# NilFoundation/crypto3-zk

Measured on AMD Instinct MI355X. Metric: MSM Mpoints/sec, BLS12-381 G1 Pippenger, 2^20 points per GPU, higher is better.
Workload: dtype u32; 1 GPU; BLS12-381 G1 Pippenger MSM, ONE MSM of 1 x 2^20 random points/scalars, bases resident; points_per_gpu=1048576, parallelism=point-range partition x1 + one all-gather of the 144-B partial sums

## Files before the change

__graft_entry__.py:

```python
import importlib.util
import os
import subprocess
import sys

ROOT = os.path.dirname(os.path.abspath(__file__))


def _load_pkg():
    if "crypto3_zk_amd" in sys.modules:
        return sys.modules["crypto3_zk_amd"]
    pkg_dir = os.path.join(ROOT, "crypto3-zk_amd")
    spec = importlib.util.spec_from_file_location("crypto3_zk_amd", os.path.join(pkg_dir, "__init__.py"),
                                                  submodule_search_locations=[pkg_dir])
    mod = importlib.util.module_from_spec(spec)
    sys.modules["crypto3_zk_amd"] = mod
    spec.loader.exec_module(mod)
    return mod


def build() -> None:
    env = dict(os.environ)
    subprocess.check_call(["make", "-C", os.path.join(ROOT, "crypto3-zk_amd"), "-j4", "all"], env=env)
    subprocess.check_call(["make", "-C", os.path.join(ROOT, "oracle"), "liboracle.so"], env=env)
    subprocess.check_call(["make", "-j2", "-C", os.path.join(ROOT, "tests", "cpp")], env=env)
    subprocess.check_call(["make", "-C", os.path.join(ROOT, "tests", "cpp"), "-f", "merkle.mk"], env=env)
    subprocess.check_call(["make", "-C", os.path.join(ROOT, "tests", "cpp"), "-f", "pow.mk"], env=env)
    subprocess.check_call(["make", "-j2", "-C", os.path.join(ROOT, "tests", "cpp"), "-f", "pasta.mk"], env=env)
    subprocess.check_call(["make", "-C", os.path.join(ROOT, "tests", "cpp"), "-f", "ipa.mk"], env=env)
    zk = _load_pkg()
    zk.load_library()


def smoke() -> None:
    import numpy as np

    sys.path.insert(0, os.path.join(ROOT, "oracle"))
    import cport as cp
    import pyoracle as po

    zk = _load_pkg()
    ctx = zk.Context(0)
    n = 5000
    ks = cp.random_fr(0, 1, n)
    bases = ctx.bases_from_scalars(zk.BLS12_381, zk.G1, ks)
    pts, inf = bases.download()
    exp_pts, _ = cp.batch_mul(0, 1, ks)
    assert (pts == exp_pts).all(), "device fixed-base multiples differ from the oracle"
    sc = cp.random_fr(0, 2, n)
    aff, is_inf = ctx.msm_affine(bases, sc)
    exp, einf = cp.msm(0, 1, pts, sc, chunks=2)
    assert is_inf == einf and (aff == exp).all(), "MSM differs from the oracle"
    grp = zk.DeviceGroup([0, 0])
    gb = grp.upload_bases(zk.BLS12_381, zk.G1, pts)
    gaff, ginf = grp.msm_affine(gb, sc)
    assert ginf == einf and (gaff == exp).all(), "device-group MSM differs from the oracle"
    gb.free()
    grp.close()
    k2 = cp.random_fr(0, 4, 300)
    b2 = ctx.bases_from_scalars(zk.BLS12_381, zk.G2, k2)
    p2, _ = b2.download()
    s2 = cp.random_fr(0, 5, 300)
    aff2, inf2 = ctx.msm_affine(b2, s2)
    exp2, einf2 = cp.msm(0, 2, p2, s2, chunks=2)
    assert inf2 == einf2 and (aff2 == exp2).all(), "G2 MSM differs from the oracle"
    b2.free()
    log_m = 12
    w = np.array(po.to_limbs(po.BLS12_381.root_of_unity(log_m), 4), dtype=np.uint64)
    a = cp.random_fr(0, 3, 2 << log_m).reshape(2, 1 << log_m, 4)
    got = ctx.ntt(zk.BLS12_381, a, log_m, w)
    assert (got == cp.ntt(0, a, log_m, w)).all(), "NTT differs from the oracle"
    assert (ctx.ntt(zk.BLS12_381, got, log_m, w, inverse=True) == a).all()
    bases.free()
    M, nin = 1024, 10
    g16 = cp.Groth16(0, M, nin, seed=3)
    kind, m = cp.domain_choice(M + nin + 1, 32)
    wd = np.array(po.to_limbs(po.BLS12_381.root_of_unity((M + nin).bit_length()), 4), dtype=np.uint64)
    gen = np.array(po.to_limbs(po.BLS12_381.fr_generator, 4), dtype=np.uint64)
    g16.set_domain(kind, m, wd)
    r1cs = ctx.upload_r1cs(zk.BLS12_381, g16.M, g16.n, g16.N, g16.csr(0), g16.csr(1), g16.csr(2))
    assert (r1cs.kind, r1cs.m) == (kind, m) == (2, 1040), "the constraint system's domain is not the reference's choice"
    z = np.concatenate([np.array([[1, 0, 0, 0]], dtype=np.uint64), g16.assignment()])
    assert (ctx.groth16_witness_h(r1cs, z, wd, gen) == g16.witness_map(wd, gen)).all(), "witness map over the step domain differs from the oracle"
    r1cs.free()
    import hashlib
    state = hashlib.sha256(b"zkhip smoke").digest()
    k = next(k for k in range(1 << 20)
             if int.from_bytes(hashlib.sha256(hashlib.sha256(state + (12345 + k).to_bytes(4, "big")).digest()).digest()[28:], "big") & 0xFFF == 0)
    assert ctx.pow_grind(state, 12345, 0xFFF) == (12345 + k, k + 1), "the device's proof of work is not the first accepted nonce"
    ctx.close()
    print("smoke ok: G1 MSM n=5000 (one context and a device group of two), G2 MSM n=300, NTT 2^12 x 2 and the witness map over a step radix-2 domain bit-exact against the oracle; proof of work (12 bits) = the reference loop's nonce")


if __name__ == "__main__":
    build()
    if len(sys.argv) > 1 and sys.argv[1] == "smoke":
        smoke()
```

crypto3-zk_amd/csrc/msm_core.hpp:

```cpp
#pragma once
#include <algorithm>
#include <string>
#include <type_traits>
#include <vector>

#ifndef ZK_NOINLINE_MUL2
#define ZK_NOINLINE_MUL2 1
#endif
#include "ctx.hpp"
#include "curve.hpp"
#include "msm_ops.hpp"
#include "msm_recode.hpp"
#include "msm_bucket_acc.hpp"
#include "fu_pair.hpp"
#include "fu_quad.hpp"

namespace {

using namespace zkhip;

constexpr uint32_t MSM_LARGE_BUCKET = 128;
constexpr uint32_t MSM_LARGE_CHUNK = 4096;
#ifndef MSM_G1_THREADS
#define MSM_G1_THREADS 64
#endif
#ifndef MSM_G2_THREADS
#define MSM_G2_THREADS 256
#endif
#ifndef MSM_G2_WAVES
#define MSM_G2_WAVES 2
#endif

template <uint32_t THREADS>
ZK_D void block_inclusive_scan(uint32_t *scratch) {
    const uint32_t t = threadIdx.x;
    __syncthreads();
    for (uint32_t d = 1; d < THREADS; d <<= 1) {
        uint32_t x = t >= d ? scratch[t - d] : 0;
        __syncthreads();
        scratch[t] += x;
        __syncthreads();
    }
}

__global__ __launch_bounds__(256) void msm_scan_local(const uint32_t *__restrict__ hist, uint32_t count, uint32_t *__restrict__ offs,
                                                      uint32_t *__restrict__ block_sums) {
    __shared__ uint32_t part[256];
    const uint32_t t = threadIdx.x, base = blockIdx.x * 1024 + t * 4;
    uint32_t v[4], s = 0;
#pragma unroll
    for (int k = 0; k < 4; ++k) {
        v[k] = base + k < count ? hist[base + k] : 0;
        s += v[k];
    }
    part[t] = s;
    block_inclusive_scan<256>(part);
    uint32_t run = part[t] - s;
#pragma unroll
    for (int k = 0; k < 4; ++k) {
        if (base + k < count) offs[base + k] = run;
        run += v[k];
    }
    if (t == 255) block_sums[blockIdx.x] = part[255];
}

__global__ __launch_bounds__(1024) void msm_scan_top(uint32_t *__restrict__ block_sums, uint32_t nblocks, uint32_t *__restrict__ total) {
    __shared__ uint32_t part[1024];
    const uint32_t t = threadIdx.x;
    const uint32_t per = (nblocks + 1023) / 1024;
    const uint32_t lo = min(nblocks, t * per), hi = min(nblocks, lo + per);
    uint32_t s = 0;
    for (uint32_t i = lo; i < hi; ++i) s += block_sums[i];
    part[t] = s;
    block_inclusive_scan<1024>(part);
    uint32_t run = part[t] - s;
    for (uint32_t i = lo; i < hi; ++i) {
        uint32_t x = block_sums[i];
        block_sums[i] = run;
        run += x;
    }
    if (t == 1023) *total = part[1023];
}

__global__ __launch_bounds__(256) void msm_scan_add(uint32_t *__restrict__ offs, uint32_t count, const uint32_t *__restrict__ block_sums,
                                                    uint32_t *__restrict__ cursor) {
    const uint32_t base = blockIdx.x * 1024 + threadIdx.x * 4;
    const uint32_t add = block_sums[blockIdx.x];
#pragma unroll
    for (int k = 0; k < 4; ++k) {
        if (base + k < count) {
            uint32_t x = offs[base + k] + add;
            offs[base + k] = x;
            cursor[base + k] = x;
        }
    }
}

__global__ __launch_bounds__(1024) void msm_scan_single(const uint32_t *__restrict__ hist, uint32_t count, uint32_t *__restrict__ offs,
                                                        uint32_t *__restrict__ cursor) {
    __shared__ uint32_t part[1024];
    __shared__ uint32_t carry;
    const uint32_t t = threadIdx.x;
    if (t == 0) carry = 0;
    __syncthreads();
    for (uint32_t base = 0; base < count; base += 1024) {
        const uint32_t v = base + t < count ? hist[base + t] : 0;
        part[t] = v;
        block_inclusive_scan<1024>(part);
        const uint32_t excl = carry + part[t] - v;
        if (base + t < count) {
            offs[base + t] = excl;
            if (cursor != offs) cursor[base + t] = excl;
        }
        __syncthreads();
        if (t == 1023) carry += part[1023];
        __syncthreads();
    }
    if (t == 0) offs[count] = carry;
}
constexpr uint32_t MSM_SCAN_SINGLE_MAX = 1u << 16;

inline int msm_scan(zkhip_ctx *ctx, const char *name, const uint32_t *hist, uint32_t count, uint32_t *offs, uint32_t *bsums) {
    if (count <= MSM_SCAN_SINGLE_MAX) {
        ZK_LAUNCH(ctx, name, msm_scan_single, dim3(1), dim3(1024), 0, hist, count, offs, offs);
        return 0;
    }
    const uint32_t nblk = (count + 1023) / 1024;
    ZK_LAUNCH(ctx, name, msm_scan_local, dim3(nblk), dim3(256), 0, hist, count, offs, bsums);
    ZK_LAUNCH(ctx, name, msm_scan_top, dim3(1), dim3(1024), 0, bsums, nblk, offs + count);
    ZK_LAUNCH(ctx, name, msm_scan_add, dim3(nblk), dim3(256), 0, offs, count, bsums, offs);
    return 0;
}

template <class FR>
__global__ __launch_bounds__(256) void msm_digits_only(const uint32_t *__restrict__ scalars, uint32_t n, MsmWindows win, uint32_t wrank,
                                                       uint32_t wworld, uint32_t *__restrict__ dig) {
    uint32_t i = blockIdx.x * blockDim.x + threadIdx.x;
    if (i >= n) return;
    uint32_t s[8];
    const uint32_t flip = msm_fold_scalar<FR>(scalars + (size_t)i * 8, s) ? 0x80000000u : 0u;
    uint32_t carry = 0, next = wrank, lw = 0;
    for (int w = 0; w < win.W; ++w) {
        uint32_t d = msm_recode(s, win.off(w), win.width(w), carry);
        if ((uint32_t)w != next) continue;
        dig[(size_t)lw * n + i] = d == DIG_NONE ? d : d ^ flip;
        next += wworld;
        ++lw;
    }
}

struct SortGeom {
    uint32_t n;
    uint32_t W;
    uint32_t B;
    uint32_t S;
    uint32_t lowb;
    uint32_t nsuper;
    uint32_t tile;
    uint32_t ntile;
    uint32_t slot0;
    uint32_t tables;
    uint32_t bases_n;
    uint32_t base_off;
};
struct SortBig {
    static constexpr uint32_t TILE = 16384, THREADS = 1024;
};
struct SortSmall {
// ... 273 lines not shown
    constexpr int NL = FieldOps<F>::WORDS;
    uint32_t g = (blockIdx.x * blockDim.x + threadIdx.x) / LPB;
    if (g >= q * B) return;
    const uint32_t s = g / B;
    uint32_t *dst = buckets + (size_t)g * (4 * NL);
    XYZZ<F> acc = xyzz_load<F>(dst);
    for (uint32_t k = 1; k < 4; ++k)
        if (s + k * q < cur) acc = xyzz_add(acc, xyzz_load<F>(buckets + ((size_t)g + (size_t)k * q * B) * (4 * NL)));
    xyzz_store<F>(dst, acc);
}

constexpr int MSM_TAIL_THREADS = 256;

template <class F>
ZK_D XYZZ<F> block_tree_sum(uint32_t *lds, XYZZ<F> acc, uint32_t t, uint32_t nthreads) {
    constexpr int NL = FieldOps<F>::WORDS;
    xyzz_store<F>(lds + (size_t)t * (4 * NL), acc);
    __syncthreads();
    for (uint32_t d = nthreads / 2; d >= 1; d >>= 1) {
        if (t < d) {
            acc = xyzz_add(xyzz_load<F>(lds + (size_t)t * (4 * NL)), xyzz_load<F>(lds + (size_t)(t + d) * (4 * NL)));
            xyzz_store<F>(lds + (size_t)t * (4 * NL), acc);
        }
        __syncthreads();
    }
    return acc;
}

template <class F, int LPB>
#ifndef ZK_TAIL_WAVES
#define ZK_TAIL_WAVES 2
#endif
__global__ __launch_bounds__(MSM_TAIL_THREADS, ZK_TAIL_WAVES) void msm_bucket_red(const uint32_t *__restrict__ buckets, uint32_t B, uint32_t L, uint32_t nseg,
                                                                   uint32_t nblk, uint32_t *__restrict__ partial) {
    constexpr int NL = FieldOps<F>::WORDS;
    extern __shared__ __attribute__((aligned(16))) uint32_t lds[];
    constexpr uint32_t SLOTS = MSM_TAIL_THREADS / LPB;
    const uint32_t t = threadIdx.x / LPB, w = blockIdx.x / nblk, seg = (blockIdx.x % nblk) * SLOTS + t;
    XYZZ<F> sum = XYZZ<F>::infinity();
    if (seg < nseg) {
        const uint32_t *base = buckets + ((size_t)w * B + (size_t)seg * L) * (4 * NL);
        if (L == 1) {
            sum = xyzz_mul_small(xyzz_load<F>(base), seg + 1);
        } else {
            XYZZ<F> run = XYZZ<F>::infinity();
            for (int b = (int)L - 1; b >= 0; --b) {
                run = xyzz_add(run, xyzz_load<F>(base + (size_t)b * (4 * NL)));
                sum = xyzz_add(sum, run);
            }
            if (seg != 0) sum = xyzz_add(sum, xyzz_mul_small(run, seg * L));
        }
    }
    sum = block_tree_sum<F>(lds, sum, t, SLOTS);
    if (t == 0) xyzz_store<F>(partial + (size_t)blockIdx.x * (4 * NL), sum);
}

template <class F, int LPB>
__global__ __launch_bounds__(256) void msm_window_sum(const uint32_t *__restrict__ partial, uint32_t nblk, uint32_t *__restrict__ winsum) {
    constexpr int NL = FieldOps<F>::WORDS;
    extern __shared__ __attribute__((aligned(16))) uint32_t lds[];
    const uint32_t w = blockIdx.x, t = threadIdx.x / LPB, slots = blockDim.x / LPB;
    XYZZ<F> acc = XYZZ<F>::infinity();
    for (uint32_t j = t; j < nblk; j += slots) acc = xyzz_add(acc, xyzz_load<F>(partial + ((size_t)w * nblk + j) * (4 * NL)));
    if (nblk > 1) acc = block_tree_sum<F>(lds, acc, t, slots);
    if (t == 0) xyzz_store<F>(winsum + (size_t)w * (4 * NL), acc);
}
inline uint32_t msm_window_threads(uint32_t nblk, int lanes_per_point) { return (size_t)nblk * lanes_per_point > 128 ? 256u : 64u; }

struct MsmFold {
    uint32_t B, C, R, log_c;
    uint32_t run;
    uint32_t m_row, m_col;
};
inline MsmFold msm_fold_geom(const zkhip_ctx *ctx, uint32_t B) {
    MsmFold g;
    int lb = 0;
    while ((1u << lb) < B) ++lb;
    g.B = B;
    g.log_c = (uint32_t)((lb + 1) / 2);
    g.C = 1u << g.log_c;
    g.R = B >> g.log_c;
    g.run = ctx->opt_msm_fold_run > 0 ? (uint32_t)ctx->opt_msm_fold_run : (B >= (1u << 18) ? 8u : 4u);
    g.run = std::max(1u, std::min(g.run, g.R));
    g.m_row = g.C / g.run;
    g.m_col = g.R / g.run;
    return g;
}

template <class FA, int LA, class FT, int LT>
__global__ __launch_bounds__(MSM_TAIL_THREADS, ZK_TAIL_WAVES) void msm_fold(const uint32_t *__restrict__ buckets, MsmFold g, uint32_t *__restrict__ level2) {
    constexpr int NL = FieldOps<FA>::WORDS;
    constexpr uint32_t SA = MSM_TAIL_THREADS / LA, ST = MSM_TAIL_THREADS / LT, PW = 4 * NL;
    extern __shared__ __attribute__((aligned(16))) uint32_t lds[];
    const uint32_t half_wgs = g.B / (SA * g.run);
    const uint32_t w = blockIdx.x / (2 * half_wgs), k = blockIdx.x % (2 * half_wgs);
    const bool col = k >= half_wgs;
    const uint32_t wg = col ? k - half_wgs : k, s = threadIdx.x / LA;
    const uint32_t m = col ? g.m_col : g.m_row, G = SA / m;
    uint32_t first, stride, slot;
    if (!col) {
        first = (wg * G + s / m) * g.C + s % m;
        stride = m;
        slot = s;
    } else {
        const uint32_t j = s / G, ll = s % G;
        first = j * g.C + wg * G + ll;
        stride = m * g.C;
        slot = ll * m + j;
    }
    {
        const uint32_t *src = buckets + ((size_t)w * g.B + first) * PW;
        XYZZ<FA> acc = xyzz_load<FA>(src);
        for (uint32_t i = 1; i < g.run; ++i) acc = xyzz_add(acc, xyzz_load<FA>(src + (size_t)i * stride * PW));
        xyzz_store<FA>(lds + (size_t)slot * PW, acc);
    }
    __syncthreads();
    const uint32_t t = threadIdx.x / LT;
    for (uint32_t half = m / 2; half >= 1; half >>= 1) {
        const uint32_t adds = G * half;
        for (uint32_t idx = t; idx < adds; idx += ST) {
            uint32_t *p = lds + (size_t)((idx / half) * m + idx % half) * PW;
            xyzz_store<FT>(p, xyzz_add(xyzz_load<FT>(p), xyzz_load<FT>(p + (size_t)half * PW)));
        }
        __syncthreads();
    }
    for (uint32_t i = t; i < G; i += ST) {
        const uint32_t o = wg * G + i;
        if (col || o != 0)
            xyzz_store<FT>(level2 + (((size_t)2 * w + (col ? 0 : 1)) * g.C + (col ? o : o - 1)) * PW, xyzz_load<FT>(lds + (size_t)i * m * PW));
    }
}

template <class F>
ZK_D void xyzz_store_canonical_jacobian(uint32_t *dst, const XYZZ<F> &p) {
    constexpr int CW = FieldOps<F>::CANON_WORDS;
    Jacobian<F> j = xyzz_to_jacobian(p);
    FieldOps<F>::to_canonical(dst, j.X);
    FieldOps<F>::to_canonical(dst + CW, j.Y);
    FieldOps<F>::to_canonical(dst + 2 * CW, j.Z);
}

template <class F, int LPB>
__global__ __launch_bounds__(64) void msm_final_fold(const uint32_t *__restrict__ winsum, uint32_t count, uint32_t shift, uint32_t *const *__restrict__ outs,
                                                     uint32_t *__restrict__ out) {
    constexpr int NL = FieldOps<F>::WORDS;
    if (blockIdx.x >= count || threadIdx.x >= LPB) return;
    XYZZ<F> acc = xyzz_load<F>(winsum + ((size_t)2 * blockIdx.x + 1) * (4 * NL));
    if (!acc.is_inf())
        for (uint32_t i = 0; i < shift; ++i) acc = xyzz_dbl(acc);
    acc = xyzz_add(acc, xyzz_load<F>(winsum + (size_t)2 * blockIdx.x * (4 * NL)));
    xyzz_store_canonical_jacobian<F>(outs ? outs[blockIdx.x] : out, acc);
}

template <class F, int LPB>
__global__ __launch_bounds__(64) void msm_final(const uint32_t *__restrict__ winsum, int W, MsmWindows win, uint32_t *__restrict__ out_jac) {
    constexpr int NL = FieldOps<F>::WORDS;
    if (blockIdx.x != 0 || threadIdx.x >= LPB) return;
    XYZZ<F> acc = XYZZ<F>::infinity();
    for (int w = W - 1; w >= 0; --w) {
        if (!acc.is_inf())
            for (int i = 0; i < win.width(w); ++i) acc = xyzz_dbl(acc);
        acc = xyzz_add(acc, xyzz_load<F>(winsum + (size_t)w * (4 * NL)));
    }
    xyzz_store_canonical_jacobian<F>(out_jac, acc);
}

template <class F>
__global__ __launch_bounds__(256) void bases_to_mont(const uint32_t *__restrict__ canon, const uint8_t *__restrict__ inf, uint32_t n,
                                                     uint32_t *__restrict__ pts) {
    typedef FieldOps<F> O;
    uint32_t i = blockIdx.x * blockDim.x + threadIdx.x;
    if (i >= n) return;
    const uint32_t *c = canon + (size_t)i * (2 * O::CANON_WORDS);
    Affine<F> a;
    if (inf != nullptr && inf[i]) a = Affine<F>::infinity();
    else a = {O::from_canonical(c), O::from_canonical(c + O::CANON_WORDS)};
    affine_store<F>(pts + (size_t)i * (2 * O::WORDS), a);
}

template <class F>
__global__ __launch_bounds__(256) void bases_from_mont(const uint32_t *__restrict__ pts, uint32_t n, uint32_t *__restrict__ out,
                                                       uint8_t *__restrict__ inf) {
    typedef FieldOps<F> O;
    uint32_t i = blockIdx.x * blockDim.x + threadIdx.x;
    if (i >= n) return;
    Affine<F> a = affine_load<F>(pts + (size_t)i * (2 * O::WORDS));
    inf[i] = a.is_inf() ? 1 : 0;
    uint32_t *o = out + (size_t)i * (2 * O::CANON_WORDS);
    O::to_canonical(o, a.x);
    O::to_canonical(o + O::CANON_WORDS, a.y);
}

template <class F>
__global__ __launch_bounds__(64) void bases_mul(uint32_t *__restrict__ pts, const uint32_t *__restrict__ base_canonical,
                                                const uint32_t *__restrict__ scalars, uint32_t n) {
    constexpr int NL = FieldOps<F>::WORDS;
    uint32_t i = blockIdx.x * blockDim.x + threadIdx.x;
    if (i >= n) return;
    Affine<F> g = {FieldOps<F>::from_canonical(base_canonical), FieldOps<F>::from_canonical(base_canonical + FieldOps<F>::CANON_WORDS)};
    const uint32_t *s = scalars + (size_t)i * 8;
    XYZZ<F> acc = XYZZ<F>::infinity();
    for (int b = 255; b >= 0; --b) {
        acc = xyzz_dbl(acc);
        if ((s[b >> 5] >> (b & 31)) & 1) acc = xyzz_madd(acc, g);
    }
    affine_store<F>(pts + (size_t)i * (2 * NL), xyzz_to_affine(acc));
}

constexpr int FIXED_WBITS = 8, FIXED_NW = 32, FIXED_ROW = 1 << FIXED_WBITS;
template <class F>
__global__ __launch_bounds__(64) void bases_fixed_table(const uint32_t *__restrict__ base_canonical, uint32_t *__restrict__ tab, uint32_t *__restrict__ tmp) {
    typedef FieldOps<F> O;
    constexpr int NL = O::WORDS;
    const uint32_t w = blockIdx.x * blockDim.x + threadIdx.x;
    if (w >= FIXED_NW) return;
    Affine<F> g = {O::from_canonical(base_canonical), O::from_canonical(base_canonical + O::CANON_WORDS)};
    XYZZ<F> P = XYZZ<F>::from_affine(g);
    for (uint32_t k = 0; k < w * FIXED_WBITS; ++k) P = xyzz_dbl(P);
    uint32_t *mine = tmp + (size_t)w * FIXED_ROW * (5 * NL);
    XYZZ<F> acc = P;
    F pre = F::one();
    for (uint32_t d = 1; d < FIXED_ROW; ++d) {
        if (d > 1) acc = xyzz_add(acc, P);
        uint32_t *slot = mine + (size_t)d * (5 * NL);
        xyzz_store<F>(slot, acc);
        pre = O::mul(pre, O::mul(acc.ZZ, acc.ZZZ));
        O::store(slot + 4 * NL, pre);
    }
    F inv = O::inv(pre);
    for (uint32_t d = FIXED_ROW; d-- > 1;) {
        const uint32_t *slot = mine + (size_t)d * (5 * NL);
        XYZZ<F> q = xyzz_load<F>(slot);
        F before = d > 1 ? O::load(mine + (size_t)(d - 1) * (5 * NL) + 4 * NL) : F::one();
        F dinv = O::mul(inv, before);
        inv = O::mul(inv, O::mul(q.ZZ, q.ZZZ));
        Affine<F> a = {O::mul(q.X, O::mul(dinv, q.ZZZ)), O::mul(q.Y, O::mul(dinv, q.ZZ))};
        affine_store<F>(tab + ((size_t)w * FIXED_ROW + d) * (2 * NL), a);
    }
}
constexpr uint32_t FIXED_CHUNK = 8;
template <class F>
__global__ __launch_bounds__(64) void bases_mul_fixed(uint32_t *__restrict__ pts, const uint32_t *__restrict__ tab, const uint32_t *__restrict__ scalars,
                                                      uint32_t n, uint32_t *__restrict__ tmp) {
    typedef FieldOps<F> O;
    constexpr int NL = O::WORDS;
    const uint32_t lo = (blockIdx.x * blockDim.x + threadIdx.x) * FIXED_CHUNK;
    if (lo >= n) return;
    const uint32_t cnt = n - lo < FIXED_CHUNK ? n - lo : FIXED_CHUNK;
    F pre = F::one();
    for (uint32_t k = 0; k < cnt; ++k) {
        const uint32_t *s = scalars + (size_t)(lo + k) * 8;
        XYZZ<F> acc = XYZZ<F>::infinity();
        for (uint32_t w = 0; w < FIXED_NW; ++w) {
            const uint32_t d = (s[w >> 2] >> ((w & 3) * 8)) & 0xFFu;
            if (d) acc = xyzz_madd(acc, affine_load<F>(tab + ((size_t)w * FIXED_ROW + d) * (2 * NL)));
        }
        uint32_t *slot = tmp + (size_t)(lo + k) * (5 * NL);
        xyzz_store<F>(slot, acc);
        if (!acc.is_inf()) pre = O::mul(pre, O::mul(acc.ZZ, acc.ZZZ));
        O::store(slot + 4 * NL, pre);
    }
    F inv = O::inv(pre);
    for (uint32_t k = cnt; k-- > 0;) {
        const uint32_t *slot = tmp + (size_t)(lo + k) * (5 * NL);
        XYZZ<F> q = xyzz_load<F>(slot);
        if (q.is_inf()) {
            affine_store<F>(pts + (size_t)(lo + k) * (2 * NL), Affine<F>::infinity());
            continue;
        }
        F before = k > 0 ? O::load(tmp + (size_t)(lo + k - 1) * (5 * NL) + 4 * NL) : F::one();
        F dinv = O::mul(inv, before);
        inv = O::mul(inv, O::mul(q.ZZ, q.ZZZ));
        Affine<F> a = {O::mul(q.X, O::mul(dinv, q.ZZZ)), O::mul(q.Y, O::mul(dinv, q.ZZ))};
        affine_store<F>(pts + (size_t)(lo + k) * (2 * NL), a);
    }
}

template <class F>
__global__ __launch_bounds__(64) void bases_precompute_range(uint32_t *__restrict__ pts, uint32_t n, uint32_t lo, uint32_t cnt, MsmWindows win,
                                                             uint32_t wrank, uint32_t wworld, uint32_t *__restrict__ tmp) {
    const int W = win.W;
    typedef FieldOps<F> O;
    constexpr int NL = O::WORDS;
    uint32_t j = blockIdx.x * blockDim.x + threadIdx.x;
    if (j >= cnt) return;
    const uint32_t i = lo + j;
    const uint32_t extra = wrank != 0 ? 1u : 0u;
    auto slot_ptr = [&](uint32_t w) { return pts + ((size_t)(w / wworld + extra) * n + i) * (2 * NL); };
    Affine<F> p = affine_load<F>(pts + (size_t)i * (2 * NL));
    if (p.is_inf()) {
        for (uint32_t w = (wrank != 0 ? wrank : wworld); w < (uint32_t)W; w += wworld) affine_store<F>(slot_ptr(w), Affine<F>::infinity());
        return;
    }
    XYZZ<F> acc = XYZZ<F>::from_affine(p);
    F pre = F::one();
    uint32_t kept = 0;
    for (int w = 1; w < W; ++w) {
        for (int k = 0; k < win.width(w - 1); ++k) acc = xyzz_dbl(acc);
        if ((uint32_t)w % wworld != wrank) continue;
        uint32_t *slot = tmp + ((size_t)kept * cnt + j) * (5 * NL);
        xyzz_store<F>(slot, acc);
        pre = O::mul(pre, O::mul(acc.ZZ, acc.ZZZ));
        O::store(slot + 4 * NL, pre);
        ++kept;
    }
    if (kept == 0) return;
    F inv = O::inv(pre);
    uint32_t w = ((uint32_t)(W - 1) - wrank) / wworld * wworld + wrank;
    for (uint32_t k = kept; k-- > 0; w -= wworld) {
        const uint32_t *slot = tmp + ((size_t)k * cnt + j) * (5 * NL);
        XYZZ<F> q = xyzz_load<F>(slot);
        F before = k > 0 ? O::load(tmp + ((size_t)(k - 1) * cnt + j) * (5 * NL) + 4 * NL) : F::one();
        F dinv = O::mul(inv, before);
        inv = O::mul(inv, O::mul(q.ZZ, q.ZZZ));
        Affine<F> a = {O::mul(q.X, O::mul(dinv, q.ZZZ)), O::mul(q.Y, O::mul(dinv, q.ZZ))};
        affine_store<F>(slot_ptr(w), a);
    }
}

template <class F>
__global__ void jac_to_affine_k(const uint32_t *__restrict__ jac, uint32_t *__restrict__ aff, uint8_t *__restrict__ inf) {
    typedef FieldOps<F> O;
    constexpr int CW = O::CANON_WORDS;
    if (blockIdx.x != 0 || threadIdx.x != 0) return;
    Jacobian<F> j = {O::from_canonical(jac), O::from_canonical(jac + CW), O::from_canonical(jac + 2 * CW)};
    XYZZ<F> q = xyzz_from_jacobian(j);
    inf[0] = q.is_inf() ? 1 : 0;
    Affine<F> a = xyzz_to_affine(q);
    O::to_canonical(aff, a.x);
    O::to_canonical(aff + CW, a.y);
}

template <class F>
__global__ void jac_sum_k(const uint32_t *__restrict__ jac, uint32_t count, uint32_t *__restrict__ out) {
    typedef FieldOps<F> O;
    constexpr int CW = O::CANON_WORDS;
    if (blockIdx.x != 0 || threadIdx.x != 0) return;
    XYZZ<F> acc = XYZZ<F>::infinity();
    for (uint32_t i = 0; i < count; ++i) {
        const uint32_t *p = jac + (size_t)i * 3 * CW;
        Jacobian<F> j = {O::from_canonical(p), O::from_canonical(p + CW), O::from_canonical(p + 2 * CW)};
        acc = xyzz_add(acc, xyzz_from_jacobian(j));
    }
    Jacobian<F> r = xyzz_to_jacobian(acc);
    O::to_canonical(out, r.X);
    O::to_canonical(out + CW, r.Y);
    O::to_canonical(out + 2 * CW, r.Z);
}

template <class F>
__global__ void msm_write_infinity(uint32_t *out_jac) {
    if (blockIdx.x != 0 || threadIdx.x != 0) return;
    xyzz_store_canonical_jacobian<F>(out_jac, XYZZ<F>::infinity());
}

template <class F, int LPB>
__global__ __launch_bounds__(64) void msm_final_batch(const uint32_t *__restrict__ winsum, uint32_t count, uint32_t *const *__restrict__ outs) {
    constexpr int NL = FieldOps<F>::WORDS;
    constexpr int CW = FieldOps<F>::CANON_WORDS;
    if (blockIdx.x >= count || threadIdx.x >= LPB) return;
    Jacobian<F> j = xyzz_to_jacobian(xyzz_load<F>(winsum + (size_t)blockIdx.x * (4 * NL)));
    uint32_t *out = outs[blockIdx.x];
    FieldOps<F>::to_canonical(out, j.X);
    FieldOps<F>::to_canonical(out + CW, j.Y);
    FieldOps<F>::to_canonical(out + 2 * CW, j.Z);
}


inline uint32_t msm_tail_segment(const zkhip_ctx *ctx, uint32_t B, size_t sets, int lanes_per_point) {
    uint32_t L = 1;
    if (ctx->opt_msm_segment_log >= 0) L = 1u << std::min(ctx->opt_msm_segment_log, 8);
    else {
        const size_t lanes = sets * B * (size_t)lanes_per_point;
        while (L < 16 && lanes / L > 65536) L <<= 1;
        while (L < 64 && lanes / L > 262144) L <<= 1;
    }
    return std::min(B, L);
}

struct MsmTailGeom {
    uint32_t L, nseg;
    uint32_t slots, nblk;
    uint32_t wthreads;
    size_t lds_red, lds_win;
};
template <class Lane>
MsmTailGeom msm_tail_geom(const zkhip_ctx *ctx, uint32_t B, size_t sets) {
    constexpr size_t point_bytes = (size_t)4 * FieldOps<typename Lane::type>::WORDS * 4;
    constexpr int XL = Lane::LANES;
    MsmTailGeom t;
    t.L = msm_tail_segment(ctx, B, sets, XL);
    t.nseg = B / t.L;
    t.slots = MSM_TAIL_THREADS / XL;
    t.nblk = (t.nseg + t.slots - 1) / t.slots;
    t.wthreads = msm_window_threads(t.nblk, XL);
    t.lds_red = t.slots * point_bytes;
    t.lds_win = t.wthreads / XL * point_bytes;
    return t;
}

template <class Lane, class Final>
int msm_tail(zkhip_ctx *ctx, const uint32_t *sets, size_t nsets, uint32_t B, uint32_t *segsum, size_t segsum_blocks, uint32_t *winsum, Final final) {
    typedef typename Lane::type TX;
    constexpr int XL = Lane::LANES;
    const MsmTailGeom t = msm_tail_geom<Lane>(ctx, B, nsets);
    if (nsets * t.nblk > segsum_blocks) {
        ctx->last_error = "MSM tail of " + std::to_string(nsets * t.nblk) + " workgroups over a partial-sum buffer for " + std::to_string(segsum_blocks);
        return ZKHIP_ERR_RANGE;
    }
    ZK_MAX_LDS(ctx, (msm_bucket_red<TX, XL>), t.lds_red);
    ZK_LAUNCH(ctx, "msm_bucket_red", (msm_bucket_red<TX, XL>), dim3((unsigned)(nsets * t.nblk)), dim3(MSM_TAIL_THREADS), t.lds_red, sets, B, t.L, t.nseg, t.nblk,
              segsum);
    ZK_LAUNCH(ctx, "msm_window_sum", (msm_window_sum<TX, XL>), dim3((unsigned)nsets), dim3(t.wthreads), t.lds_win, segsum, t.nblk, winsum);
    return final();
}

template <class F>
bool msm_fold_applies(const zkhip_ctx *ctx, uint32_t B, bool tables) {
    if (FieldOps<F>::WORDS > 16 && !ctx->opt_msm_tail_fold_g2) return false;
    if (!tables || ctx->opt_msm_tail_fold <= 0 || B < (1u << std::min(ctx->opt_msm_tail_fold, 30))) return false;
    const MsmFold g = msm_fold_geom(ctx, B);
    const uint32_t sa = MSM_TAIL_THREADS / BucketLane<F>::LANES;
    return g.m_col >= 1 && g.m_row <= sa && g.m_col <= sa && B >= sa * g.run && g.m_row * g.run == g.C && g.m_col * g.run == g.R;
}
template <class F>
struct MsmFoldBuffers {
    static constexpr size_t PW = (size_t)4 * FieldOps<F>::WORDS;
    MsmFold g{};
    size_t nsets = 0;
    uint32_t *level2 = nullptr, *segsum = nullptr, *winsum = nullptr;
    MsmFoldBuffers() = default;
    MsmFoldBuffers(const zkhip_ctx *ctx, uint32_t B, size_t nsets_) : g(msm_fold_geom(ctx, B)), nsets(nsets_) {}
    size_t level2_words() const { return nsets * 2 * g.C * PW; }
    size_t segsum_blocks() const { return nsets * 2 * ((g.C + 63) / 64); }
    template <class Arena>
    void layout(Arena &a) {
        a.take(level2, level2_words());
        a.take(segsum, segsum_blocks() * PW);
        a.take(winsum, nsets * 2 * PW);
    }
};

template <class F, class Lane>
int msm_fold_tail(zkhip_ctx *ctx, const uint32_t *sets, const MsmFoldBuffers<F> &fb, uint32_t *const *d_outs, uint32_t *d_out) {
    constexpr int NL = FieldOps<F>::WORDS;
    typedef typename BucketLane<F>::type FL;
    constexpr int LPB = BucketLane<F>::LANES;
    typedef typename QuadLane<F>::type TQ;
    constexpr int QL = QuadLane<F>::LANES;
    const MsmFold &g = fb.g;
    const size_t nsets = fb.nsets;
    ZK_HIP_CHECK(ctx, hipMemsetAsync(fb.level2, 0, fb.level2_words() * 4, ctx->stream));
    const size_t lds = (size_t)MSM_TAIL_THREADS / LPB * 4 * NL * 4;
    ZK_MAX_LDS(ctx, (msm_fold<FL, LPB, TQ, QL>), lds);
    ZK_LAUNCH(ctx, "msm_fold", (msm_fold<FL, LPB, TQ, QL>), dim3((unsigned)(nsets * (g.B / (MSM_TAIL_THREADS / LPB * g.run)) * 2)), dim3(MSM_TAIL_THREADS), lds,
              sets, g, fb.level2);
    auto level2 = [&](auto lane) -> int {
        typedef decltype(lane) X;
        return msm_tail<X>(ctx, fb.level2, 2 * nsets, g.C, fb.segsum, fb.segsum_blocks(), fb.winsum, [&]() -> int {
            ZK_LAUNCH(ctx, "msm_final", (msm_final_fold<typename X::type, X::LANES>), dim3((unsigned)nsets), dim3(64), 0, fb.winsum, (uint32_t)nsets, g.log_c, d_outs, d_out);
            return 0;
        });
    };
    if (QuadLane<F>::AVAILABLE && ctx->opt_msm_tail_quads && 2 * nsets * g.C <= ((size_t)1 << 18)) return level2(QuadLane<F>());
    return level2(Lane());
}

struct MsmPlan {
    int c, W_all, W;
    uint32_t B, S, nb;
    MsmWindows win;
    uint32_t wrank, wworld;
    bool tables;
};

inline MsmPlan msm_plan(const zkhip_ctx *ctx, const zkhip_bases *bases, size_t n) {
    MsmPlan p;
    p.tables = bases->tables();
    int c = p.tables ? bases->c_tab : ctx->opt_msm_window_bits;
    if (c <= 0) c = zk_msm_auto_window(n);
    p.c = std::max(2, std::min(ZK_MSM_MAX_C, c));
    if (!p.tables) p.c = std::min(p.c, 16);
    p.W_all = msm_windows(zk_scalar_bits(bases->curve), p.c);
    p.win = msm_make_windows(zk_scalar_bits(bases->curve), p.W_all);
    p.wrank = p.tables ? (uint32_t)bases->win_rank : 0u;
    p.wworld = p.tables ? (uint32_t)bases->win_world : 1u;
    p.W = p.tables ? bases->local_windows() : p.W_all;
    p.B = 1u << (p.c - 1);
    if (!p.tables) p.S = (uint32_t)p.W;
    else {
        int s = ctx->opt_msm_sets;
        if (s <= 0) s = (int)((zk_msm_target_lanes() + p.B - 1) / p.B);
        p.S = (uint32_t)std::max(1, std::min(p.W, s));
        while (p.S > 1 && (uint64_t)p.S * p.B > ((uint64_t)SORT_MAX_SUPER << SORT_MAX_LOW)) --p.S;
    }
    p.nb = p.S * p.B;
    return p;
}

template <class SZ>
int msm_sort_run(zkhip_ctx *ctx, const SortGeom &g, uint32_t nbh, const uint32_t *dig, uint32_t *bh, uint32_t *bo, uint32_t *bsums, uint32_t *tmp_idx,
                 uint16_t *tmp_key, uint32_t *offs, uint32_t *idx) {
    const size_t lds_hist = (size_t)g.nsuper * 4;
    const size_t lds_split = ((size_t)3 * g.nsuper + 1 + SZ::THREADS + 2 * SZ::TILE) * 4;
    const size_t lds_final = (size_t)SZ::TILE * 6;
    if (lds_split > 48 * 1024) ZK_MAX_LDS(ctx, msm_sort_split<SZ>, 160 * 1024 - 256);
    if (lds_final > 40 * 1024) ZK_MAX_LDS(ctx, msm_sort_final<SZ>, 160 * 1024 - (4 * SORT_NLOW_MAX + SZ::THREADS) * 4 - 256);
    ZK_LAUNCH(ctx, "msm_sort_hist", msm_sort_hist<SZ>, dim3(g.ntile, g.W), dim3(SZ::THREADS), lds_hist, dig, g, bh);
    ZK_TRY(msm_scan(ctx, "msm_scan", bh, nbh, bo, bsums));
    ZK_LAUNCH(ctx, "msm_sort_split", msm_sort_split<SZ>, dim3(g.ntile, g.W), dim3(SZ::THREADS), lds_split, dig, g, bo, tmp_idx, tmp_key);
    ZK_LAUNCH(ctx, "msm_sort_final", msm_sort_final<SZ>, dim3(g.nsuper), dim3(SZ::THREADS), lds_final, tmp_idx, tmp_key, g, g.S * g.B, bo, offs, idx);
    return 0;
}

struct MsmCall {
    MsmPlan P;
    SortGeom g;
    bool big_tiles;
    uint32_t nbh;
    uint32_t sblk, nsh;
    int Sr;
    uint32_t segsum_blocks;
    bool fold;
    uint32_t large_thresh, large_cap, task_cap;
    size_t entries() const { return (size_t)P.W * g.n; }
};

template <class F>
int msm_call_plan(const zkhip_ctx *ctx, const zkhip_bases *bases, size_t offset, size_t n, bool batch_member, MsmCall &c, std::string &error) {
    const MsmPlan &P = c.P = msm_plan(ctx, bases, n);
    if ((uint64_t)P.W * n >= (1ull << 32) || (uint64_t)bases->nslots * bases->n >= (1ull << 31)) {
        error = "MSM of " + std::to_string(n) + " points x " + std::to_string(P.W) + " windows exceeds the 32-bit entry index (split the range)";
        return ZKHIP_ERR_RANGE;
    }
    SortGeom &g = c.g;
    g.n = (uint32_t)n;
    g.W = (uint32_t)P.W;
    g.B = P.B;
    g.S = P.S;
    g.lowb = (uint32_t)std::min<int>(SORT_MAX_LOW, P.c - 1);
    g.nsuper = (P.nb + (1u << g.lowb) - 1) >> g.lowb;
    c.big_tiles = ctx->opt_msm_sort_tile_log >= 14;
    g.tile = c.big_tiles ? SortBig::TILE : SortSmall::TILE;
    g.ntile = (uint32_t)((n + g.tile - 1) / g.tile);
    g.tables = P.tables ? 1u : 0u;
    g.slot0 = P.tables ? (uint32_t)bases->slot_of_local(0) : 0u;
    g.bases_n = (uint32_t)bases->n;
    g.base_off = (uint32_t)offset;
    if (g.nsuper > SORT_MAX_SUPER) return ZKHIP_ERR_RANGE;
    const size_t nbh64 = (size_t)g.nsuper * g.W * g.ntile;
    if (nbh64 >= (1ull << 31)) return ZKHIP_ERR_RANGE;
    c.nbh = (uint32_t)nbh64;
    c.sblk = (P.nb + 1023) / 1024;
    c.nsh = SIZE_BINS * c.sblk;
    c.Sr = P.tables ? 1 : P.W;
    c.segsum_blocks = std::max(msm_tail_geom<TailLane<F>>(ctx, P.B, c.Sr).nblk, msm_tail_geom<QuadLane<F>>(ctx, P.B, c.Sr).nblk);
    c.fold = !batch_member && msm_fold_applies<F>(ctx, P.B, P.tables);
    c.large_thresh = (uint32_t)std::max<size_t>(MSM_LARGE_BUCKET, 4 * ((c.entries() + P.nb - 1) / P.nb));
    c.large_cap = (uint32_t)(c.entries() / c.large_thresh + 1);
    c.task_cap = (uint32_t)(c.entries() / MSM_LARGE_CHUNK + c.large_cap + 1);
    return 0;
}

template <class F>
struct MsmBuffers {
    static constexpr size_t PW = (size_t)4 * FieldOps<F>::WORDS;
    const MsmCall &c;
    uint32_t *dig, *bh, *bo, *bsums, *tmp_idx;
    uint16_t *tmp_key;
    uint32_t *offs, *idx, *buckets;
    uint32_t *sh, *so, *ssums, *order;
    uint32_t *segsum, *winsum;
    MsmFoldBuffers<F> fb;
    uint32_t *plan, *tasks, *large, *partials;
    MsmBuffers(const zkhip_ctx *ctx, const MsmCall &call) : c(call) {
        if (c.fold) fb = MsmFoldBuffers<F>(ctx, c.P.B, 1);
    }
    template <class Arena>
    void layout(Arena &a) {
        a.take(dig, c.entries());
        a.take(bh, c.nbh);
        a.take(bo, (size_t)c.nbh + 1);
        a.take(bsums, (c.nbh + 1023) / 1024);
        a.take(tmp_idx, c.entries());
        a.take(tmp_key, c.entries());
        a.take(offs, (size_t)c.P.nb + 1);
        a.take(idx, c.entries());
        a.take(buckets, c.P.nb * PW);
        a.take(sh, (size_t)c.nsh + 1);
        a.take(so, (size_t)c.nsh + 1);
        a.take(ssums, (c.nsh + 1023) / 1024);
        a.take(order, c.P.nb);
        a.take(segsum, (size_t)c.Sr * c.segsum_blocks * PW);
        a.take(winsum, (size_t)std::max(1, c.Sr) * PW);
        if (c.fold) fb.layout(a);
        a.take(plan, 4);
        a.take(tasks, (size_t)c.task_cap * 3);
        a.take(large, (size_t)c.large_cap * 3);
        a.take(partials, c.task_cap * PW);
    }
};

template <class F>
int msm_stages(zkhip_ctx *ctx, const zkhip_bases *bases, const MsmCall &c, const MsmBuffers<F> &w, const uint32_t *d_scalars, bool reuse_sort) {
    constexpr int NL = FieldOps<F>::WORDS;
    typedef typename BucketLane<F>::type FL;
    constexpr int LPB = BucketLane<F>::LANES;
    const MsmPlan &P = c.P;
    const uint32_t n = c.g.n, nb = P.nb;
    const uint32_t *d_b = bases->d;
    if (!reuse_sort) {
        ZK_TRY(fr_sat_dispatch(bases->curve, [&](auto fr) -> int {
            typedef typename decltype(fr)::type FR;
            ZK_LAUNCH(ctx, "msm_digits", msm_digits_only<FR>, grid_1d(n), dim3(256), 0, d_scalars, n, P.win, P.wrank, P.wworld, w.dig);
            return 0;
        }));
// ... 241 lines not shown
```

Measured before the change: 383.4 Mpoints/s.

## Add wavefront-wide XYZZ arithmetic for the single-set MSM fold tail

Adds a new point representation that spreads one XYZZ point across a full 64-lane wavefront, one 16-lane DPP row per coordinate. Field multiplication uses DPP broadcasts and carry normalisation uses ballot-based carry lookahead. The second-level MSM tail (bucket weighting, tree reduction and final fold) is replaced by new wide kernels when there is one set and quad tails are enabled. The aim is to cut the latency of the serial tail reduction by using far more lanes per point addition. The cost is heavy cross-lane traffic and a slow fallback for the doubling case.

```diff
diff --git a/__graft_entry__.py b/__graft_entry__.py
--- a/__graft_entry__.py
+++ b/__graft_entry__.py
@@ -26,6 +26,7 @@
     subprocess.check_call(["make", "-C", os.path.join(ROOT, "tests", "cpp"), "-f", "merkle.mk"], env=env)
     subprocess.check_call(["make", "-C", os.path.join(ROOT, "tests", "cpp"), "-f", "pow.mk"], env=env)
     subprocess.check_call(["make", "-j2", "-C", os.path.join(ROOT, "tests", "cpp"), "-f", "pasta.mk"], env=env)
+    subprocess.check_call(["make", "-C", os.path.join(ROOT, "tests", "cpp"), "-f", "wide.mk"], env=env)
     subprocess.check_call(["make", "-C", os.path.join(ROOT, "tests", "cpp"), "-f", "ipa.mk"], env=env)
     zk = _load_pkg()
     zk.load_library()
diff --git a/crypto3-zk_amd/csrc/fu_wide.hpp b/crypto3-zk_amd/csrc/fu_wide.hpp
--- /dev/null
+++ b/crypto3-zk_amd/csrc/fu_wide.hpp
@@ -0,0 +1,217 @@
+#pragma once
+#include <utility>
+
+#include "fu_quad.hpp"
+
+namespace zkhip {
+
+template <class U>
+struct FuW {
+    typedef U params;
+};
+
+ZK_D uint32_t wide_lane() { return __builtin_amdgcn_mbcnt_hi(~0u, __builtin_amdgcn_mbcnt_lo(~0u, 0u)); }
+ZK_D uint32_t wide_row() { return wide_lane() >> 4; }
+
+template <class U>
+struct XYZZ<FuW<U>> {
+    uint32_t w;
+    ZK_D bool is_inf() const { return ((uint32_t)(__builtin_amdgcn_ballot_w64(w == 0) >> 32) & 0xffffu) == 0xffffu; }
+    ZK_D static XYZZ infinity() { return {0u}; }
+};
+
+template <class U, class Fn>
+ZK_D uint32_t wide_const(Fn f) {
+    const uint32_t j = wide_lane() & 15u;
+    uint32_t r = 0;
+#pragma unroll
+    for (int i = 0; i < U::L; ++i) r = j == (uint32_t)i ? f(i) : r;
+    return r;
+}
+template <class U>
+ZK_D uint32_t wide_mod() { return wide_const<U>([](int i) { return U::mod(i); }); }
+
+template <int CTRL>
+ZK_D uint32_t wide_dpp(uint32_t x) {
+    uint32_t r = (uint32_t)__builtin_amdgcn_update_dpp(0, (int)x, CTRL, 0xF, 0xF, true);
+    asm volatile("" : "+v"(r));
+    return r;
+}
+template <int I>
+ZK_D uint32_t wide_bcast(uint32_t x) { return wide_dpp<0x150 + I>(x); }
+ZK_D uint32_t wide_down(uint32_t x) { return wide_dpp<0x101>(x); }
+ZK_D uint32_t wide_up(uint32_t x) { return wide_dpp<0x111>(x); }
+
+template <int S0, int S1, int S2, int S3>
+ZK_D uint32_t wide_rows(uint32_t x) {
+    constexpr uint32_t PACK = (uint32_t)(S0 | (S1 << 2) | (S2 << 4) | (S3 << 6));
+    const uint32_t lane = wide_lane();
+    const uint32_t src = (((PACK >> (2 * (lane >> 4))) & 3u) << 4) | (lane & 15u);
+    return (uint32_t)__builtin_amdgcn_ds_bpermute((int)(src << 2), (int)x);
+}
+ZK_D uint32_t wide_pick(uint32_t x0, uint32_t x1, uint32_t x2, uint32_t x3) {
+    const uint32_t lane = wide_lane();
+    const bool b0 = (lane & 16u) != 0, b1 = (lane & 32u) != 0;
+    return b1 ? (b0 ? x3 : x2) : (b0 ? x1 : x0);
+}
+
+template <class U>
+ZK_D uint32_t wide_norm(uint32_t v) {
+    constexpr int L = U::L, B = U::B;
+    constexpr uint32_t MASK = Fu<U>::MASK;
+    static_assert(L <= 15, "lane 15 of a row ends the carry chain");
+    constexpr uint64_t LOW = (((uint64_t)1 << (L - 1)) - 1) * 0x0001000100010001ull;
+    const bool low = (wide_lane() & 15u) < (uint32_t)(L - 1);
+    const uint32_t lm = low ? MASK : 0xffffffffu;
+    const uint32_t v1 = (v & lm) + wide_up(v >> (low ? B : 31));
+    const uint64_t G = __builtin_amdgcn_ballot_w64(v1 > MASK) & LOW, P = __builtin_amdgcn_ballot_w64(v1 == MASK) & LOW;
+    const uint64_t cin = ((G | P) + G) ^ P;
+    uint32_t r;
+    uint64_t cout;
+    asm("v_addc_co_u32_e64 %0, %1, %2, 0, %3" : "=v"(r), "=s"(cout) : "v"(v1), "s"(cin));
+    return r & lm;
+}
+
+template <class U>
+ZK_D uint32_t wide_add(uint32_t a, uint32_t b) { return wide_norm<U>(a + b); }
+template <int K, class U>
+ZK_D uint32_t wide_sub(uint32_t a, uint32_t b) {
+    const uint32_t s = wide_const<U>([](int i) { return U::template spread<K>(i); });
+    return wide_norm<U>(a + (s - b));
+}
+
+template <int L, int... I>
+ZK_D void wide_bcast_all(uint32_t a, uint32_t (&ai)[L], std::integer_sequence<int, I...>) {
+    ((ai[I] = wide_bcast<I>(a)), ...);
+}
+template <class U>
+ZK_D uint32_t wide_mul(uint32_t a, uint32_t b) {
+    constexpr int L = U::L, B = U::B;
+    constexpr uint32_t MASK = Fu<U>::MASK;
+    static_assert(B == 29, "the column bounds are those of 29-bit limbs");
+    const uint32_t p = wide_mod<U>();
+    uint32_t ai[L];
+    wide_bcast_all(a, ai, std::make_integer_sequence<int, L>());
+    uint32_t t = 0;
+#pragma unroll
+    for (int i = 0; i < L; ++i) {
+        uint64_t acc = (uint64_t)ai[i] * b + t;
+        const uint32_t q = (wide_bcast<0>((uint32_t)acc) * U::QINV) & MASK;
+        acc += (uint64_t)q * p;
+        t = (uint32_t)(acc >> B) + wide_down((uint32_t)acc & MASK);
+    }
+    return wide_norm<U>(t);
+}
+
+template <class U>
+ZK_D XYZZ<FuQ<U>> wide_gather(const XYZZ<FuW<U>> &a) {
+    XYZZ<FuQ<U>> r;
+    Fu<U> *c[4] = {&r.X.v, &r.Y.v, &r.ZZ.v, &r.ZZZ.v};
+#pragma unroll
+    for (int k = 0; k < 4; ++k) {
+#pragma unroll
+        for (int i = 0; i < U::L; ++i) c[k]->v[i] = (uint32_t)__builtin_amdgcn_readlane((int)a.w, 16 * k + i);
+    }
+    return r;
+}
+template <class U>
+ZK_D XYZZ<FuW<U>> wide_scatter(const XYZZ<FuQ<U>> &a) {
+    const Fu<U> *c[4] = {&a.X.v, &a.Y.v, &a.ZZ.v, &a.ZZZ.v};
+    uint32_t x[4];
+#pragma unroll
+    for (int k = 0; k < 4; ++k) x[k] = wide_const<U>([&](int i) { return c[k]->v[i]; });
+    return {wide_pick(x[0], x[1], x[2], x[3])};
+}
+
+template <class U>
+ZK_D XYZZ<FuW<U>> wide_load(const uint32_t *p) {
+    static_assert(U::L <= 15 && U::SL <= 16 && U::L <= U::SL, "a coordinate is one DPP row");
+    const uint32_t lane = wide_lane(), j = lane & 15u;
+    return {j < (uint32_t)U::L ? p[(lane >> 4) * U::SL + j] : 0u};
+}
+template <class U>
+ZK_D void wide_store(uint32_t *p, const XYZZ<FuW<U>> &a) {
+    static_assert(U::L <= 15 && U::SL <= 16 && U::L <= U::SL, "a coordinate is one DPP row");
+    const uint32_t lane = wide_lane(), j = lane & 15u;
+    if (j < (uint32_t)U::SL) p[(lane >> 4) * U::SL + j] = a.w;
+}
+
+template <class U>
+__device__ __noinline__ uint32_t wide_add_whole(uint32_t a, uint32_t b) {
+    return wide_scatter<U>(xyzz_add(wide_gather<U>(XYZZ<FuW<U>>{a}), wide_gather<U>(XYZZ<FuW<U>>{b}))).w;
+}
+
+template <class U>
+ZK_D XYZZ<FuW<U>> xyzz_dbl(const XYZZ<FuW<U>> &a) {
+    typedef FieldOps<Fu<U>> O;
+    if (a.is_inf()) return XYZZ<FuW<U>>::infinity();
+    const uint32_t row = wide_row();
+    const uint32_t a2 = wide_add<U>(a.w, a.w);
+    const uint32_t o1 = row == 0 ? a.w : wide_rows<1, 1, 1, 1>(a2);
+    const uint32_t s1 = wide_mul<U>(o1, o1);
+    const uint32_t M = wide_norm<U>(s1 + s1 + s1);
+    const uint32_t s2 = wide_mul<U>(wide_pick(M, a2, a.w, wide_rows<0, 0, 0, 0>(a.w)), row == 0 ? M : s1);
+    const uint32_t sw = wide_rows<3, 1, 1, 1>(s2);
+    const uint32_t X3 = wide_sub<O::K1, U>(s2, wide_add<U>(sw, sw));
+    const uint32_t D = wide_sub<O::K2, U>(sw, X3);
+    const uint32_t s3 = wide_mul<U>(row == 0 ? M : (row == 1 ? s2 : a.w), wide_pick(D, a.w, a.w, sw));
+    const uint32_t Y3 = wide_sub<O::K1, U>(wide_rows<0, 0, 0, 0>(s3), s3);
+    return {wide_pick(X3, Y3, s2, s3)};
+}
+
+template <class U>
+ZK_D XYZZ<FuW<U>> xyzz_add(const XYZZ<FuW<U>> &a, const XYZZ<FuW<U>> &b) {
+    typedef FieldOps<Fu<U>> O;
+    if (a.is_inf()) return b;
+    if (b.is_inf()) return a;
+    const uint32_t row = wide_row();
+    const uint32_t s1 = wide_mul<U>(a.w, wide_rows<2, 3, 0, 1>(b.w));
+    const uint32_t T = wide_sub<O::K1, U>(wide_rows<2, 3, 2, 3>(s1), s1);
+    const uint32_t s2 = wide_mul<U>(row < 2 ? T : a.w, row < 2 ? T : b.w);
+    {
+        const uint32_t z = (uint32_t)__builtin_amdgcn_ballot_w64(s2 == 0) & 0xffffu, e = (uint32_t)__builtin_amdgcn_ballot_w64(s2 == wide_mod<U>()) & 0xffffu;
+        if (z == 0xffffu || e == 0xffffu) return {wide_add_whole<U>(a.w, b.w)};
+    }
+    const uint32_t sx = wide_rows<1, 0, 0, 0>(s1);
+    const uint32_t s3 = wide_mul<U>(wide_pick(T, sx, s2, s2), wide_rows<0, 0, 0, 0>(s2));
+    const uint32_t PPP = wide_rows<0, 0, 0, 0>(s3);
+    const uint32_t X3 = wide_sub<O::K1, U>(s2, wide_norm<U>(PPP + s3 + s3));
+    const uint32_t D = wide_sub<O::K2, U>(s3, X3);
+    const uint32_t s4 = wide_mul<U>(wide_pick(sx, D, s2, s2), row == 1 ? T : PPP);
+    const uint32_t Y3 = wide_sub<O::K1, U>(s4, wide_rows<0, 0, 0, 0>(s4));
+    return {wide_pick(wide_rows<1, 1, 1, 1>(X3), Y3, s3, s4)};
+}
+
+template <class U>
+ZK_D XYZZ<FuW<U>> xyzz_mul_small(const XYZZ<FuW<U>> &a, uint32_t k) {
+    XYZZ<FuW<U>> r = XYZZ<FuW<U>>::infinity();
+    if (k == 0 || a.is_inf()) return r;
+    int top = 31;
+    while (!((k >> top) & 1)) --top;
+    r = a;
+    for (int i = top - 1; i >= 0; --i) {
+        r = xyzz_dbl(r);
+        if ((k >> i) & 1) r = xyzz_add(r, a);
+    }
+    return r;
+}
+
+template <class F>
+struct WideLane {
+    static constexpr bool AVAILABLE = false;
+    typedef typename TailLane<F>::type type;
+    static constexpr int LANES = TailLane<F>::LANES;
+};
+template <class U>
+struct WideLane<Fu<U>> {
+    static constexpr bool AVAILABLE = true;
+    typedef FuW<U> type;
+    static constexpr int LANES = 64;
+    ZK_D static XYZZ<type> xyzz_load(const uint32_t *p) { return wide_load<U>(p); }
+    ZK_D static void xyzz_store(uint32_t *p, const XYZZ<type> &a) { wide_store<U>(p, a); }
+    ZK_D static XYZZ<type> xyzz_add(const XYZZ<type> &a, const XYZZ<type> &b) { return zkhip::xyzz_add(a, b); }
+    ZK_D static XYZZ<type> xyzz_dbl(const XYZZ<type> &a) { return zkhip::xyzz_dbl(a); }
+    ZK_D static XYZZ<type> xyzz_mul_small(const XYZZ<type> &a, uint32_t k) { return zkhip::xyzz_mul_small(a, k); }
+};
+
+}
diff --git a/crypto3-zk_amd/csrc/msm_core.hpp b/crypto3-zk_amd/csrc/msm_core.hpp
--- a/crypto3-zk_amd/csrc/msm_core.hpp
+++ b/crypto3-zk_amd/csrc/msm_core.hpp
@@ -14,6 +14,7 @@
 #include "msm_bucket_acc.hpp"
 #include "fu_pair.hpp"
 #include "fu_quad.hpp"
+#include "fu_wide.hpp"
 
 namespace {
 
@@ -593,6 +594,62 @@
     xyzz_store_canonical_jacobian<F>(outs ? outs[blockIdx.x] : out, acc);
 }
 
+constexpr uint32_t MSM_WIDE_WAVES = 8;
+
+template <class U>
+ZK_D XYZZ<FuW<U>> wide_tree_sum(uint32_t *lds, XYZZ<FuW<U>> acc, uint32_t w, uint32_t nw) {
+    constexpr uint32_t PW = 4 * U::SL;
+    wide_store<U>(lds + w * PW, acc);
+    __syncthreads();
+    for (uint32_t d = nw / 2; d >= 1; d >>= 1) {
+        if (w < d) {
+            acc = xyzz_add(wide_load<U>(lds + w * PW), wide_load<U>(lds + (w + d) * PW));
+            wide_store<U>(lds + w * PW, acc);
+        }
+        __syncthreads();
+    }
+    return acc;
+}
+
+template <class U>
+__global__ __launch_bounds__(MSM_WIDE_WAVES * 64) void msm_wide_weigh(const uint32_t *__restrict__ points, uint32_t C, uint32_t *__restrict__ partial) {
+    constexpr uint32_t PW = 4 * U::SL;
+    __shared__ uint32_t lds[MSM_WIDE_WAVES * PW];
+    const uint32_t w = threadIdx.x >> 6, i = blockIdx.x * MSM_WIDE_WAVES + w;
+    XYZZ<FuW<U>> acc = xyzz_mul_small(wide_load<U>(points + (size_t)i * PW), (i & (C - 1)) + 1);
+    acc = wide_tree_sum<U>(lds, acc, w, MSM_WIDE_WAVES);
+    if (w == 0) wide_store<U>(partial + (size_t)blockIdx.x * PW, acc);
+}
+
+template <class U>
+__global__ __launch_bounds__(MSM_WIDE_WAVES * 64) void msm_wide_tree(const uint32_t *__restrict__ in, uint32_t *__restrict__ out) {
+    constexpr uint32_t PW = 4 * U::SL;
+    __shared__ uint32_t lds[MSM_WIDE_WAVES * PW];
+    const uint32_t w = threadIdx.x >> 6;
+    const uint32_t *src = in + ((size_t)blockIdx.x * 2 * MSM_WIDE_WAVES + w) * PW;
+    XYZZ<FuW<U>> acc = xyzz_add(wide_load<U>(src), wide_load<U>(src + (size_t)MSM_WIDE_WAVES * PW));
+    acc = wide_tree_sum<U>(lds, acc, w, MSM_WIDE_WAVES);
+    if (w == 0) wide_store<U>(out + (size_t)blockIdx.x * PW, acc);
+}
+
+template <class U>
+__global__ __launch_bounds__(MSM_WIDE_WAVES * 64) void msm_wide_final(const uint32_t *__restrict__ partial, uint32_t m, uint32_t shift, uint32_t *const *__restrict__ outs,
+                                                                      uint32_t *__restrict__ out) {
+    constexpr uint32_t PW = 4 * U::SL, HALF = MSM_WIDE_WAVES / 2;
+    __shared__ uint32_t lds[MSM_WIDE_WAVES * PW];
+    const uint32_t w = threadIdx.x >> 6, half = w / HALF, q = w % HALF;
+    const uint32_t *src = partial + ((size_t)2 * blockIdx.x + (1 - half)) * m * PW;
+    XYZZ<FuW<U>> acc = XYZZ<FuW<U>>::infinity();
+    for (uint32_t j = q; j < m; j += HALF) acc = xyzz_add(acc, wide_load<U>(src + (size_t)j * PW));
+    acc = wide_tree_sum<U>(lds + half * HALF * PW, acc, q, HALF);
+    if (w != 0) return;
+    if (!acc.is_inf())
+        for (uint32_t i = 0; i < shift; ++i) acc = xyzz_dbl(acc);
+    acc = xyzz_add(acc, wide_load<U>(lds + HALF * PW));
+    const XYZZ<FuQ<U>> whole = wide_gather<U>(acc);
+    if (wide_lane() < 4) xyzz_store_canonical_jacobian<FuQ<U>>(outs ? outs[blockIdx.x] : out, whole);
+}
+
 template <class F, int LPB>
 __global__ __launch_bounds__(64) void msm_final(const uint32_t *__restrict__ winsum, int W, MsmWindows win, uint32_t *__restrict__ out_jac) {
     constexpr int NL = FieldOps<F>::WORDS;
@@ -873,7 +930,7 @@
     MsmFoldBuffers() = default;
     MsmFoldBuffers(const zkhip_ctx *ctx, uint32_t B, size_t nsets_) : g(msm_fold_geom(ctx, B)), nsets(nsets_) {}
     size_t level2_words() const { return nsets * 2 * g.C * PW; }
-    size_t segsum_blocks() const { return nsets * 2 * ((g.C + 63) / 64); }
+    size_t segsum_blocks() const { return nsets * 2 * std::max<size_t>((g.C + 63) / 64, WideLane<F>::AVAILABLE && nsets == 1 ? g.C / MSM_WIDE_WAVES : 0); }
     template <class Arena>
     void layout(Arena &a) {
         a.take(level2, level2_words());
@@ -881,6 +938,37 @@
         a.take(winsum, nsets * 2 * PW);
     }
 };
+
+template <class F>
+bool msm_tail_wide_applies(const zkhip_ctx *ctx, size_t nsets, uint32_t C) {
+    return WideLane<F>::AVAILABLE && ctx->opt_msm_tail_quads == 1 && nsets == 1 && C >= MSM_WIDE_WAVES;
+}
+template <class F>
+int msm_tail_wide(zkhip_ctx *ctx, const MsmFoldBuffers<F> &fb, uint32_t *const *d_outs, uint32_t *d_out) {
+    if constexpr (WideLane<F>::AVAILABLE) {
+        typedef typename F::params U;
+        const uint32_t C = fb.g.C;
+        const size_t sets = 2 * fb.nsets;
+        uint32_t m = C / MSM_WIDE_WAVES;
+        if (sets * m > fb.segsum_blocks()) {
+            ctx->last_error = "wide MSM tail of " + std::to_string(sets * m) + " workgroups over a partial-sum buffer for " + std::to_string(fb.segsum_blocks());
+            return ZKHIP_ERR_RANGE;
+        }
+        uint32_t *from = fb.segsum, *to = fb.level2;
+        ZK_LAUNCH(ctx, "msm_wide_weigh", (msm_wide_weigh<U>), dim3((unsigned)(sets * m)), dim3(MSM_WIDE_WAVES * 64), 0, fb.level2, C, from);
+        while (m > MSM_WIDE_WAVES) {
+            m /= 2 * MSM_WIDE_WAVES;
+            ZK_LAUNCH(ctx, "msm_wide_tree", (msm_wide_tree<U>), dim3((unsigned)(sets * m)), dim3(MSM_WIDE_WAVES * 64), 0, from, to);
+            std::swap(from, to);
+        }
+        ZK_LAUNCH(ctx, "msm_wide_final", (msm_wide_final<U>), dim3((unsigned)fb.nsets), dim3(MSM_WIDE_WAVES * 64), 0, from, m, fb.g.log_c, d_outs, d_out);
+        return 0;
+    } else {
+        (void)fb, (void)d_outs, (void)d_out;
+        ctx->last_error = "no wide lane for this field";
+        return ZKHIP_ERR_INVALID;
+    }
+}
 
 template <class F, class Lane>
 int msm_fold_tail(zkhip_ctx *ctx, const uint32_t *sets, const MsmFoldBuffers<F> &fb, uint32_t *const *d_outs, uint32_t *d_out) {
@@ -903,6 +991,7 @@
             return 0;
         });
     };
+    if (msm_tail_wide_applies<F>(ctx, nsets, g.C)) return msm_tail_wide<F>(ctx, fb, d_outs, d_out);
     if (QuadLane<F>::AVAILABLE && ctx->opt_msm_tail_quads && 2 * nsets * g.C <= ((size_t)1 << 18)) return level2(QuadLane<F>());
     return level2(Lane());
 }
```

New measurement: 403.2 Mpoints/s (median of 6 runs). 5.2% higher.
